# arianna011/Audio-ResiDual

Hardware: NVIDIA B200
Metric: htsat_residual_clips_per_sec (higher is better)
Workload: dtype bf16

## Files before the change

### audio_residual_b200/csrc/ard_common.cuh

```cuda
#pragma once
#include <cuda_runtime.h>
#include <cuda_bf16.h>
#include <cuda_fp16.h>
#include <cuda.h>
#include <stdint.h>

#define ARD_DEVINL __device__ __forceinline__

namespace ard {

ARD_DEVINL uint32_t smem_u32(const void* p) { return static_cast<uint32_t>(__cvta_generic_to_shared(p)); }

ARD_DEVINL uint32_t elect_one_sync() {
    uint32_t pred = 0;
    asm volatile(
        "{\n\t.reg .pred P1;\n\t.reg .b32 R1;\n\t"
        "elect.sync R1|P1, 0xffffffff;\n\t"
        "selp.u32 %0, 1, 0, P1;\n\t}\n"
        : "=r"(pred));
    return pred;
}

ARD_DEVINL uint32_t pack_bf16x2(float lo, float hi) {
    uint32_t r;
// ... 145 lines not shown
}

constexpr uint32_t PAIR_LEADER_MASK = 0xFEFFFFFFu;
ARD_DEVINL uint32_t cluster_ctarank() {
    uint32_t r;
    asm volatile("mov.u32 %0, %%cluster_ctarank;" : "=r"(r));
    return r;
}
ARD_DEVINL void cluster_sync_all() {
    asm volatile("barrier.cluster.arrive.release.aligned;\n\tbarrier.cluster.wait.acquire.aligned;" ::: "memory");
}
ARD_DEVINL void tma_load_2d_pair(void* smem_dst, const CUtensorMap* m, uint64_t* bar, int c0, int c1) {
    asm volatile(
        "cp.async.bulk.tensor.2d.cta_group::2.shared::cluster.global.mbarrier::complete_tx::bytes [%0], [%1, {%3, %4}], [%2];"
        ::"r"(smem_u32(smem_dst)), "l"(reinterpret_cast<uint64_t>(m)), "r"(smem_u32(bar) & PAIR_LEADER_MASK), "r"(c0), "r"(c1)
        : "memory");
}
ARD_DEVINL void tmem_alloc_pair(uint32_t* smem_dst, uint32_t ncols) {
    asm volatile("tcgen05.alloc.cta_group::2.sync.aligned.shared::cta.b32 [%0], %1;" ::"r"(smem_u32(smem_dst)), "r"(ncols)
                 : "memory");
}
ARD_DEVINL void tmem_relinquish_pair() { asm volatile("tcgen05.relinquish_alloc_permit.cta_group::2.sync.aligned;" ::: "memory"); }
ARD_DEVINL void tmem_dealloc_pair(uint32_t taddr, uint32_t ncols) {
    asm volatile("tcgen05.dealloc.cta_group::2.sync.aligned.b32 %0, %1;" ::"r"(taddr), "r"(ncols) : "memory");
}
ARD_DEVINL void umma_bf16_ss_pair(uint32_t tmem_d, uint64_t desc_a, uint64_t desc_b, uint32_t idesc, uint32_t accumulate) {
    asm volatile(
        "{\n\t.reg .pred p;\n\t"
        "setp.ne.b32 p, %4, 0;\n\t"
        "tcgen05.mma.cta_group::2.kind::f16 [%0], %1, %2, %3, p;\n\t}\n"
        ::"r"(tmem_d), "l"(desc_a), "l"(desc_b), "r"(idesc), "r"(accumulate)
        : "memory");
}
ARD_DEVINL void umma_commit_pair(uint64_t* bar) {
    asm volatile("tcgen05.commit.cta_group::2.mbarrier::arrive::one.shared::cluster.multicast::cluster.b64 [%0], %1;"
                 ::"r"(smem_u32(bar)), "h"((uint16_t)3)
                 : "memory");
}
ARD_DEVINL void mbar_arrive_leader(uint64_t* bar) {
    asm volatile("mbarrier.arrive.release.cluster.shared::cluster.b64 _, [%0];" ::"r"(smem_u32(bar) & PAIR_LEADER_MASK) : "memory");
}
ARD_DEVINL void mbar_wait_cluster(uint64_t* bar, uint32_t parity) {
    uint32_t ok = 0;
    while (!ok) {
        asm volatile(
            "{\n\t.reg .pred p;\n\t"
            "mbarrier.try_wait.parity.acquire.cluster.shared::cta.b64 p, [%1], %2;\n\t"
            "selp.u32 %0, 1, 0, p;\n\t}\n"
            : "=r"(ok)
            : "r"(smem_u32(bar)), "r"(parity)
            : "memory");
    }
}

ARD_DEVINL void tmem_ld_32x32b_x32(uint32_t taddr, uint32_t (&v)[32]) {
    asm volatile(
        "tcgen05.ld.sync.aligned.32x32b.x32.b32 "
        "{%0, %1, %2, %3, %4, %5, %6, %7, %8, %9, %10, %11, %12, %13, %14, %15, "
        "%16, %17, %18, %19, %20, %21, %22, %23, %24, %25, %26, %27, %28, %29, %30, %31}, [%32];"
        : "=r"(v[0]), "=r"(v[1]), "=r"(v[2]), "=r"(v[3]), "=r"(v[4]), "=r"(v[5]), "=r"(v[6]), "=r"(v[7]), "=r"(v[8]),
          "=r"(v[9]), "=r"(v[10]), "=r"(v[11]), "=r"(v[12]), "=r"(v[13]), "=r"(v[14]), "=r"(v[15]), "=r"(v[16]),
          "=r"(v[17]), "=r"(v[18]), "=r"(v[19]), "=r"(v[20]), "=r"(v[21]), "=r"(v[22]), "=r"(v[23]), "=r"(v[24]),
          "=r"(v[25]), "=r"(v[26]), "=r"(v[27]), "=r"(v[28]), "=r"(v[29]), "=r"(v[30]), "=r"(v[31])
        : "r"(taddr)
        : "memory");
}
ARD_DEVINL void tmem_ld_32x32b_x16(uint32_t taddr, uint32_t (&v)[16]) {
    asm volatile(
        "tcgen05.ld.sync.aligned.32x32b.x16.b32 "
        "{%0, %1, %2, %3, %4, %5, %6, %7, %8, %9, %10, %11, %12, %13, %14, %15}, [%16];"
        : "=r"(v[0]), "=r"(v[1]), "=r"(v[2]), "=r"(v[3]), "=r"(v[4]), "=r"(v[5]), "=r"(v[6]), "=r"(v[7]), "=r"(v[8]),
          "=r"(v[9]), "=r"(v[10]), "=r"(v[11]), "=r"(v[12]), "=r"(v[13]), "=r"(v[14]), "=r"(v[15])
        : "r"(taddr)
        : "memory");
}
ARD_DEVINL void tmem_ld_32x32b_x8(uint32_t taddr, uint32_t (&v)[8]) {
    asm volatile("tcgen05.ld.sync.aligned.32x32b.x8.b32 {%0, %1, %2, %3, %4, %5, %6, %7}, [%8];"
                 : "=r"(v[0]), "=r"(v[1]), "=r"(v[2]), "=r"(v[3]), "=r"(v[4]), "=r"(v[5]), "=r"(v[6]), "=r"(v[7])
                 : "r"(taddr)
                 : "memory");
}
ARD_DEVINL void tmem_ld_wait() { asm volatile("tcgen05.wait::ld.sync.aligned;" ::: "memory"); }

ARD_DEVINL uint64_t umma_desc_sw128(uint32_t smem_addr) {
    uint64_t d = 0;
    d |= (uint64_t)((smem_addr & 0x3FFFF) >> 4);
    d |= (uint64_t)1 << 16;
    d |= (uint64_t)(1024 >> 4) << 32;
    d |= (uint64_t)1 << 46;
    d |= (uint64_t)2 << 61;
    return d;
}
ARD_DEVINL uint64_t umma_desc_sw64(uint32_t smem_addr) {
    uint64_t d = 0;
    d |= (uint64_t)((smem_addr & 0x3FFFF) >> 4);
    d |= (uint64_t)1 << 16;
    d |= (uint64_t)(512 >> 4) << 32;
    d |= (uint64_t)1 << 46;
    d |= (uint64_t)4 << 61;
    return d;
}
__host__ __device__ constexpr uint32_t umma_idesc_bf16(int M, int N) {
    return (1u << 4) | (1u << 7) | (1u << 10) | ((uint32_t)(N >> 3) << 17) | ((uint32_t)(M >> 4) << 24);
}
__host__ __device__ constexpr uint32_t umma_idesc_f16(int M, int N) {
    return (1u << 4) | ((uint32_t)(N >> 3) << 17) | ((uint32_t)(M >> 4) << 24);
// ... 48 lines not shown
```

### audio_residual_b200/csrc/ffn_wide.cu

```cuda
#include "ard_common.cuh"
#include "ard_internal.h"

namespace ard {

#ifdef ARD_FFN_TRACE
__device__ long long g_ffw_trace[8][64][8];
#define FW_TRACE(role, idx, field) do { if (blockIdx.x == 0 && (idx) < 64) g_ffw_trace[role][idx][field] = clock64(); } while (0)
#else
#define FW_TRACE(role, idx, field) do { } while (0)
#endif

constexpr int FW_BM = 128;
constexpr int FW_EPI_WARPS = 8;
constexpr int FW_GELU_WARPS = 16;
constexpr int FW_W_MMA = FW_EPI_WARPS, FW_W_TMA = FW_W_MMA + 1, FW_W_GELU = FW_W_TMA + 1, FW_W_MMA2 = FW_W_GELU + FW_GELU_WARPS;
constexpr int FW_THREADS = (FW_W_MMA2 + 1) * 32;
constexpr int FW_TM_H = 384;

template <int C>
struct FwCfg {
    static_assert(C == 128 || C == 192 || C == 256 || C == 384, "ffn_wide: C = 128, 192, 256 or 384");
    static constexpr int HD = 4 * C;
    static constexpr int NCH = HD / 64;
    static constexpr int YW = (C % 192 == 0) ? 192 : C;
    static constexpr int KBS = YW / 64;
    static constexpr int SLOT = YW * 128;
    static constexpr int NS = C / YW;
    static constexpr int KB1 = C / 64;
    static constexpr int NYB = 1;
    static constexpr bool A2T = C <= 256;
    static constexpr int TM_A2 = C;
    static constexpr int NA1 = 1;
    static constexpr int NSLOT = C == 128 ? 8 : C == 192 ? 5 : 3;
    static constexpr int A1_KB = FW_BM * 128;
    static constexpr int A1_OFF = 0;
    static constexpr int A1_BYTES = KB1 * A1_KB;
    static constexpr int A2_OFF = A1_OFF + NA1 * A1_BYTES;
    static constexpr int A2_BYTES = FW_BM * 128;
    static constexpr int RING_OFF = A2_OFF + 2 * A2_BYTES;
    static constexpr int CST_OFF = RING_OFF + NSLOT * SLOT;
    static constexpr int VEC_OFF = CST_OFF + FW_EPI_WARPS * 2048;
    static constexpr int BAR_OFF = VEC_OFF + 3 * C * 4;
    static constexpr int SMEM_BYTES = BAR_OFF + 384 + 1024;
    static_assert(SMEM_BYTES <= 227 * 1024, "ffn_wide: shared memory budget");
    static constexpr int LN_CH = C / 16;
    static constexpr int LN_V4 = LN_CH / 4;
    static constexpr int LN_STEPS = LN_CH <= 12 ? 4 : 2;
};

struct FwParams {
    const float* x;
    const float* resid2;
    const float* gamma;
    const float* beta;
    const float* b1h;
    const float* b2;
    int M;
};

template <int C>
__global__ void __launch_bounds__(FW_THREADS, 1)
ffn_wide_kernel(const __grid_constant__ CUtensorMap tmW1, const __grid_constant__ CUtensorMap tmW2,
                const __grid_constant__ CUtensorMap tmOut, const __grid_constant__ CUtensorMap tmX,
                const __grid_constant__ CUtensorMap tmR2, const FwParams p) {
    using Cfg = FwCfg<C>;
    constexpr int NCH = Cfg::NCH, NS = Cfg::NS, NSLOT = Cfg::NSLOT, NYB = Cfg::NYB, NA1 = Cfg::NA1;
    extern __shared__ uint8_t smem_raw[];
    uint8_t* smem = smem_raw + ((1024u - (smem_u32(smem_raw) & 1023u)) & 1023u);
    float* b2s = reinterpret_cast<float*>(smem + Cfg::VEC_OFF);
    float* gs = b2s + C;
    float* bs = gs + C;
    uint64_t* bars = reinterpret_cast<uint64_t*>(smem + Cfg::BAR_OFF);
    uint64_t* ring_full = bars + 0;
    uint64_t* ring_empty = bars + 8;
    uint64_t* a1_full = bars + 16;
    uint64_t* a1_free = bars + 18;
    uint64_t* h_full = bars + 20;
    uint64_t* h_free = bars + 22;
    uint64_t* a2_full = bars + 24;
    uint64_t* a2_free = bars + 26;
    uint64_t* y_full = bars + 28;
    uint64_t* y_free = bars + 30;
    uint32_t* tmem_ptr_smem = reinterpret_cast<uint32_t*>(bars + 32);
    uint64_t* rbar = bars + 34;

    pdl_launch_dependents();
    const int warp = threadIdx.x >> 5, lane = threadIdx.x & 31;
    const int num_tiles = (p.M + FW_BM - 1) / FW_BM;
    const int my_tiles = (num_tiles - (int)blockIdx.x + (int)gridDim.x - 1) / (int)gridDim.x;

    for (int i = threadIdx.x; i < C; i += FW_THREADS) {
        b2s[i] = p.b2[i];
        gs[i] = p.gamma[i];
        bs[i] = p.beta[i];
    }
    if (warp == FW_W_MMA && lane == 0) {
        tma_prefetch_desc(&tmW1);
        tma_prefetch_desc(&tmW2);
        tma_prefetch_desc(&tmOut);
        for (int i = 0; i < NSLOT; ++i) {
            mbar_init(&ring_full[i], 1);
            mbar_init(&ring_empty[i], 1);
        }
        for (int i = 0; i < 2; ++i) {
            mbar_init(&a1_full[i], FW_GELU_WARPS);
            mbar_init(&a1_free[i], 1);
            mbar_init(&h_full[i], 1);
            mbar_init(&h_free[i], FW_GELU_WARPS / 2);
            mbar_init(&a2_full[i], FW_GELU_WARPS / 2);
            mbar_init(&a2_free[i], 1);
            mbar_init(&y_full[i], 1);
            mbar_init(&y_free[i], FW_EPI_WARPS);
        }
        for (int i = 0; i < FW_EPI_WARPS; ++i) mbar_init(&rbar[i], 1);
        fence_barrier_init();
    }
    if (warp == FW_W_MMA) {
        tmem_alloc(tmem_ptr_smem, 512);
        tmem_relinquish();
    }
    tc_fence_before();
    __syncthreads();
    tc_fence_after();
    const uint32_t tmem_base = *tmem_ptr_smem;
    pdl_wait();

    if (warp < FW_EPI_WARPS) {
        constexpr int NCC = C / 32;
        const int quad = warp & 3, c_begin = (warp >> 2) * NCC;
        uint8_t* sbuf = smem + Cfg::CST_OFF + warp * 2048;
        const bool has_r2 = p.resid2 != nullptr;
        if constexpr (Cfg::A2T) {
            uint8_t* rb1 = smem + Cfg::A2_OFF + warp * 4096;
            uint8_t* rb2 = rb1 + 2048;
            auto fetch_resid = [&](int tile, int c) {
                mbar_expect_tx(&rbar[warp], has_r2 ? 4096 : 2048);
                tma_load_2d(rb1, &tmX, &rbar[warp], c * 16, tile * FW_BM + quad * 32);
                if (has_r2) tma_load_2d(rb2, &tmR2, &rbar[warp], c * 16, tile * FW_BM + quad * 32);
            };
            if (lane == 0) fetch_resid(blockIdx.x, c_begin);
            int it = 0;
            for (int tile = blockIdx.x; tile < num_tiles; tile += gridDim.x, ++it) {
                if (warp == 0 && lane == 0) FW_TRACE(0, it, 0);
                mbar_wait_parked(&y_full[0], (uint32_t)(it & 1));
                if (warp == 0 && lane == 0) FW_TRACE(0, it, 1);
                tc_fence_after();
#pragma unroll 1
                for (int cc = 0; cc < NCC; ++cc) {
                    const int c = c_begin + cc;
                    uint32_t v[16];
                    tmem_ld_32x32b_x16(tmem_base + c * 16 + ((uint32_t)(quad * 32) << 16), v);
                    mbar_wait(&rbar[warp], (uint32_t)((it * NCC + cc) & 1));
                    const int sw = (lane >> 1) & 3;
                    float4 r1[4], r2[4];
#pragma unroll
                    for (int j = 0; j < 4; ++j) {
                        r1[j] = *reinterpret_cast<const float4*>(rb1 + lane * 64 + ((j ^ sw) << 4));
                        r2[j] = has_r2 ? *reinterpret_cast<const float4*>(rb2 + lane * 64 + ((j ^ sw) << 4)) : make_float4(0.f, 0.f, 0.f, 0.f);
                    }
                    fence_proxy_async_smem();
                    __syncwarp();
                    if (lane == 0) {
                        if (cc + 1 < NCC) fetch_resid(tile, c + 1);
                        else if (tile + (int)gridDim.x < num_tiles) fetch_resid(tile + gridDim.x, c_begin);
                    }
                    tmem_ld_wait();
                    if (cc == NCC - 1) {
                        tc_fence_before();
                        __syncwarp();
                        if (lane == 0) mbar_arrive(&y_free[0]);
                    }
                    float4 o[4];
#pragma unroll
                    for (int j = 0; j < 4; ++j) {
                        const float4 b4 = *reinterpret_cast<const float4*>(b2s + c * 16 + j * 4);
                        o[j].x = __uint_as_float(v[j * 4 + 0]) + b4.x + r1[j].x + r2[j].x;
                        o[j].y = __uint_as_float(v[j * 4 + 1]) + b4.y + r1[j].y + r2[j].y;
                        o[j].z = __uint_as_float(v[j * 4 + 2]) + b4.z + r1[j].z + r2[j].z;
                        o[j].w = __uint_as_float(v[j * 4 + 3]) + b4.w + r1[j].w + r2[j].w;
                    }
                    if (lane == 0) tma_store_wait_read<0>();
                    __syncwarp();
                    uint8_t* rowp = sbuf + lane * 64;
#pragma unroll
                    for (int j = 0; j < 4; ++j) *reinterpret_cast<float4*>(rowp + ((j ^ sw) << 4)) = o[j];
                    fence_proxy_async_smem();
                    __syncwarp();
                    if (lane == 0) {
                        tma_store_2d(&tmOut, sbuf, c * 16, tile * FW_BM + quad * 32);
                        tma_store_commit();
                    }
                }
                if (warp == 0 && lane == 0) FW_TRACE(0, it, 2);
            }
        } else {
        int it = 0;
        for (int tile = blockIdx.x; tile < num_tiles; tile += gridDim.x, ++it) {
            const int yb = it % NYB;
            const uint32_t ypar = (it / NYB) & 1;
            const long long row = (long long)tile * FW_BM + quad * 32 + lane;
            const bool row_ok = row < p.M;
            float4 r1[4], r2[4];
            auto load_resid = [&](int c) {
#pragma unroll
                for (int j = 0; j < 4; ++j) { r1[j] = make_float4(0.f, 0.f, 0.f, 0.f); r2[j] = r1[j]; }
                if (row_ok) {
                    const float4* rp = reinterpret_cast<const float4*>(p.x + row * C + c * 16);
#pragma unroll
                    for (int j = 0; j < 4; ++j) r1[j] = rp[j];
                    if (has_r2) {
                        const float4* rq = reinterpret_cast<const float4*>(p.resid2 + row * C + c * 16);
#pragma unroll
                        for (int j = 0; j < 4; ++j) r2[j] = rq[j];
                    }
                }
            };
            load_resid(c_begin);
            if (warp == 0 && lane == 0) FW_TRACE(0, it, 0);
            mbar_wait_parked(&y_full[yb], ypar);
            if (warp == 0 && lane == 0) FW_TRACE(0, it, 1);
            tc_fence_after();
#pragma unroll 1
            for (int cc = 0; cc < NCC; ++cc) {
                const int c = c_begin + cc;
                uint32_t v[16];
                tmem_ld_32x32b_x16(tmem_base + yb * 192 + c * 16 + ((uint32_t)(quad * 32) << 16), v);
                tmem_ld_wait();
                if (cc == NCC - 1) {
                    tc_fence_before();
                    __syncwarp();
                    if (lane == 0) mbar_arrive(&y_free[yb]);
                }
                float4 o[4];
#pragma unroll
                for (int j = 0; j < 4; ++j) {
                    const float4 b4 = *reinterpret_cast<const float4*>(b2s + c * 16 + j * 4);
                    o[j].x = __uint_as_float(v[j * 4 + 0]) + b4.x + r1[j].x + r2[j].x;
                    o[j].y = __uint_as_float(v[j * 4 + 1]) + b4.y + r1[j].y + r2[j].y;
                    o[j].z = __uint_as_float(v[j * 4 + 2]) + b4.z + r1[j].z + r2[j].z;
                    o[j].w = __uint_as_float(v[j * 4 + 3]) + b4.w + r1[j].w + r2[j].w;
                }
                if (cc + 1 < NCC) load_resid(c + 1);
                if (lane == 0) tma_store_wait_read<0>();
                __syncwarp();
                uint8_t* rowp = sbuf + lane * 64;
                const int sw = (lane >> 1) & 3;
#pragma unroll
                for (int j = 0; j < 4; ++j) *reinterpret_cast<float4*>(rowp + ((j ^ sw) << 4)) = o[j];
                fence_proxy_async_smem();
                __syncwarp();
                if (lane == 0) {
                    tma_store_2d(&tmOut, sbuf, c * 16, tile * FW_BM + quad * 32);
                    tma_store_commit();
                }
            }
            if (warp == 0 && lane == 0) FW_TRACE(0, it, 2);
        }
        }
        if (lane == 0) tma_store_wait_all<0>();
    } else if (warp == FW_W_TMA) {
        long long n = 0;
        for (int t = 0; t < my_tiles; ++t) {
#pragma unroll 1
            for (int e = 0; e < 2 * NCH; ++e) {
                const bool is_w2 = e >= 2 && (e == 2 * NCH - 1 || (e & 1) == 0);
                const int j = e < 2 ? e : (e == 2 * NCH - 1 ? NCH - 1 : (is_w2 ? (e - 2) >> 1 : (e + 1) >> 1));
#pragma unroll 1
                for (int s = 0; s < NS; ++s, ++n) {
                    const int slot = (int)(n % NSLOT);
                    const uint32_t par = (uint32_t)((n / NSLOT) & 1);
                    if (lane == 0) FW_TRACE(6, (int)n, 0);
                    mbar_wait_parked(&ring_empty[slot], par ^ 1);
                    if (lane == 0) FW_TRACE(6, (int)n, 1);
                    if (elect_one_sync()) {
                        uint8_t* dst = smem + Cfg::RING_OFF + slot * Cfg::SLOT;
                        mbar_expect_tx(&ring_full[slot], Cfg::SLOT);
                        if (is_w2) {
                            tma_load_2d(dst, &tmW2, &ring_full[slot], j * 64, s * Cfg::YW);
                        } else {
#pragma unroll
                            for (int kb = 0; kb < Cfg::KBS; ++kb)
                                tma_load_2d(dst + kb * 8192, &tmW1, &ring_full[slot], s * Cfg::YW + kb * 64, j * 64);
                        }
                    }
                    __syncwarp();
                }
            }
        }
    } else if (warp == FW_W_MMA) {
        constexpr uint32_t idesc1 = umma_idesc_bf16(FW_BM, 64);
        const uint64_t dA1 = umma_desc_sw128(smem_u32(smem + Cfg::A1_OFF));
        const uint32_t ring_u32 = smem_u32(smem + Cfg::RING_OFF);
        long long g = 0;
        for (int t = 0; t < my_tiles; ++t) {
            const int ab = t % NA1;
            mbar_wait_parked(&a1_full[ab], (uint32_t)((t / NA1) & 1));
#pragma unroll 1
            for (int j = 0; j < NCH; ++j, ++g) {
                const int hb = j & 1;
                if (lane == 0) FW_TRACE(1, (int)g, 0);
                mbar_wait_parked(&h_free[hb], (uint32_t)(((g >> 1) & 1) ^ 1));
                if (lane == 0) FW_TRACE(1, (int)g, 1);
                tc_fence_after();
                const int e = j < 2 ? j : 2 * j - 1;
                const long long n0 = ((long long)t * 2 * NCH + e) * NS;
#pragma unroll 1
                for (int s = 0; s < NS; ++s) {
                    const long long n = n0 + s;
                    const int slot = (int)(n % NSLOT);
                    mbar_wait_parked(&ring_full[slot], (uint32_t)((n / NSLOT) & 1));
                    tc_fence_after();
                    if (elect_one_sync()) {
                        const uint32_t d = tmem_base + FW_TM_H + hb * 64;
                        const uint64_t db = umma_desc_sw128(ring_u32 + slot * Cfg::SLOT);
#pragma unroll
                        for (int kb = 0; kb < Cfg::KBS; ++kb)
                            umma_f16_ss_run<4>(d, dA1 + (uint64_t)((ab * Cfg::KB1 + s * Cfg::KBS + kb) * (Cfg::A1_KB >> 4)), db + (uint64_t)(kb * (8192 >> 4)), idesc1,
                                               (s | kb) != 0);
                        umma_commit(&ring_empty[slot]);
                        if (s == NS - 1) {
                            umma_commit(&h_full[hb]);
                            if (j == NCH - 1) umma_commit(&a1_free[ab]);
                        }
                    }
                    __syncwarp();
                    if (lane == 0) FW_TRACE(1, (int)g, 2 + s);
                }
            }
        }
    } else if (warp == FW_W_MMA2) {
        constexpr uint32_t idesc2 = umma_idesc_f16(FW_BM, Cfg::YW);
        const uint64_t dA2 = umma_desc_sw128(smem_u32(smem + Cfg::A2_OFF));
        const uint32_t ring_u32 = smem_u32(smem + Cfg::RING_OFF);
        long long g = 0;
        for (int t = 0; t < my_tiles; ++t) {
            const int yb = t % NYB;
#pragma unroll 1
            for (int j = 0; j < NCH; ++j, ++g) {
                const int b = j & 1;
                if (lane == 0) FW_TRACE(2, (int)g, 0);
                mbar_wait_parked(&a2_full[b], (uint32_t)((g >> 1) & 1));
                if (lane == 0) FW_TRACE(2, (int)g, 1);
                if (j == 0) mbar_wait_parked(&y_free[yb], (uint32_t)(((t / NYB) & 1) ^ 1));
                if (lane == 0) FW_TRACE(2, (int)g, 2);
                tc_fence_after();
                const int e = j < NCH - 1 ? 2 * j + 2 : 2 * NCH - 1;
                const long long n0 = ((long long)t * 2 * NCH + e) * NS;
#pragma unroll 1
                for (int s = 0; s < NS; ++s) {
                    const long long n = n0 + s;
                    const int slot = (int)(n % NSLOT);
                    mbar_wait_parked(&ring_full[slot], (uint32_t)((n / NSLOT) & 1));
                    tc_fence_after();
                    if (elect_one_sync()) {
                        if constexpr (Cfg::A2T)
                            umma_f16_ts_run4(tmem_base + yb * 192 + s * Cfg::YW, tmem_base + Cfg::TM_A2 + b * 32,
                                             umma_desc_sw128(ring_u32 + slot * Cfg::SLOT), idesc2, j != 0);
                        else
                            umma_f16_ss_run<4>(tmem_base + yb * 192 + s * Cfg::YW, dA2 + (uint64_t)(b * (Cfg::A2_BYTES >> 4)),
                                               umma_desc_sw128(ring_u32 + slot * Cfg::SLOT), idesc2, j != 0);
                        umma_commit(&ring_empty[slot]);
                        if (s == NS - 1) {
                            umma_commit(&a2_free[b]);
                            if (j == NCH - 1) umma_commit(&y_full[yb]);
                        }
                    }
                    __syncwarp();
                    if (lane == 0) FW_TRACE(2, (int)g, 3 + s);
                }
            }
        }
    } else {
        const int ew = warp - FW_W_GELU;
        const int quad = warp & 3;
        const int grp = ew >> 3;
        const int half = (ew >> 2) & 1;
        const int row = quad * 32 + lane;
        const int l16 = lane & 15, rsub = lane >> 4;
        uint8_t* a1 = smem + Cfg::A1_OFF;
        auto prefetch_tile = [&](int tile) {
            if (tile >= num_tiles) return;
            const long long r0 = (long long)tile * FW_BM + ew * 8;
            for (int ofs = lane * 128; ofs < 8 * C * 4; ofs += 32 * 128) {
                if ((r0 * C) * 4 + ofs + 128 > (long long)p.M * C * 4) break;
                asm volatile("prefetch.global.L2 [%0];" ::"l"(reinterpret_cast<const char*>(p.x + r0 * C) + ofs));
                if (p.resid2 != nullptr)
                    asm volatile("prefetch.global.L2 [%0];" ::"l"(reinterpret_cast<const char*>(p.resid2 + r0 * C) + ofs));
            }
        };
        auto layernorm_tile = [&](int tile, int lt) {
            prefetch_tile(tile + gridDim.x);
            constexpr int V4 = Cfg::LN_V4, STEPS = Cfg::LN_STEPS;
            bool waited = false;
#pragma unroll 1
            for (int sp = 0; sp < 4 / STEPS; ++sp) {
                float4 v[STEPS][V4];
#pragma unroll
                for (int st = 0; st < STEPS; ++st) {
                    const long long r = (long long)tile * FW_BM + ew * 8 + (sp * STEPS + st) * 2 + rsub;
                    if (r < p.M) {
                        const float4* xr = reinterpret_cast<const float4*>(p.x + r * C + l16 * Cfg::LN_CH);
#pragma unroll
                        for (int q = 0; q < V4; ++q) v[st][q] = __ldg(xr + q);
                    } else {
#pragma unroll
                        for (int q = 0; q < V4; ++q) v[st][q] = make_float4(0.f, 0.f, 0.f, 0.f);
                    }
                }
                if (!waited) {
                    if (ew == 0 && lane == 0) FW_TRACE(3, lt, 0);
                    mbar_wait_parked(&a1_free[lt % NA1], (uint32_t)(((lt / NA1) & 1) ^ 1));
                    if (ew == 0 && lane == 0) FW_TRACE(3, lt, 1);
                    waited = true;
                }
                float sm[STEPS], qv[STEPS];
#pragma unroll
                for (int st = 0; st < STEPS; ++st) {
                    sm[st] = 0.f;
#pragma unroll
                    for (int q = 0; q < V4; ++q) sm[st] += (v[st][q].x + v[st][q].y) + (v[st][q].z + v[st][q].w);
                }
#pragma unroll
                for (int sh = 8; sh > 0; sh >>= 1)
#pragma unroll
                    for (int st = 0; st < STEPS; ++st) sm[st] += __shfl_xor_sync(0xffffffffu, sm[st], sh);
#pragma unroll
                for (int st = 0; st < STEPS; ++st) {
                    const float mean = sm[st] * (1.0f / C);
                    qv[st] = 0.f;
#pragma unroll
                    for (int q = 0; q < V4; ++q) {
                        v[st][q].x -= mean; v[st][q].y -= mean; v[st][q].z -= mean; v[st][q].w -= mean;
                        qv[st] += (v[st][q].x * v[st][q].x + v[st][q].y * v[st][q].y) + (v[st][q].z * v[st][q].z + v[st][q].w * v[st][q].w);
                    }
                }
#pragma unroll
                for (int sh = 8; sh > 0; sh >>= 1)
#pragma unroll
                    for (int st = 0; st < STEPS; ++st) qv[st] += __shfl_xor_sync(0xffffffffu, qv[st], sh);
#pragma unroll
                for (int st = 0; st < STEPS; ++st) {
                    const float rstd = rsqrtf(qv[st] * (1.0f / C) + 1e-5f);
                    const int rr = ew * 8 + (sp * STEPS + st) * 2 + rsub;
#pragma unroll
                    for (int q = 0; q < V4; ++q) {
                        const int c0 = l16 * Cfg::LN_CH + q * 4;
                        const float4 gm = *reinterpret_cast<const float4*>(gs + c0);
                        const float4 bt = *reinterpret_cast<const float4*>(bs + c0);
                        uint2 pk;
                        pk.x = pack_bf16x2(fmaf(v[st][q].x * rstd, gm.x, bt.x), fmaf(v[st][q].y * rstd, gm.y, bt.y));
                        pk.y = pack_bf16x2(fmaf(v[st][q].z * rstd, gm.z, bt.z), fmaf(v[st][q].w * rstd, gm.w, bt.w));
                        const int kb = c0 >> 6, cc = c0 & 63;
                        *reinterpret_cast<uint2*>(a1 + ((lt % NA1) * Cfg::KB1 + kb) * Cfg::A1_KB + rr * 128 + (((cc >> 3) ^ (rr & 7)) << 4) + (cc & 7) * 2) = pk;
                    }
                }
            }
            fence_proxy_async_smem();
            __syncwarp();
            if (lane == 0) mbar_arrive(&a1_full[lt % NA1]);
            if (ew == 0 && lane == 0) FW_TRACE(3, lt, 2);
        };

        prefetch_tile(blockIdx.x);
        if (my_tiles > 0) layernorm_tile(blockIdx.x, 0);
        int it = 0;
        for (int tile = blockIdx.x; tile < num_tiles; tile += gridDim.x, ++it) {
#pragma unroll 1
            for (int jj = 0; jj < NCH / 2; ++jj) {
                const int j = 2 * jj + grp;
                const long long g = (long long)it * NCH + j;
                if ((ew & 7) == 0 && lane == 0) FW_TRACE(4 + grp, (int)g, 0);
                mbar_wait_parked(&h_full[grp], (uint32_t)((g >> 1) & 1));
                if ((ew & 7) == 0 && lane == 0) FW_TRACE(4 + grp, (int)g, 1);
                tc_fence_after();
                uint32_t pk[16];
#pragma unroll
                for (int s = 0; s < 2; ++s) {
                    uint32_t v[16];
                    tmem_ld_32x32b_x16(tmem_base + FW_TM_H + grp * 64 + half * 32 + s * 16 + ((uint32_t)(quad * 32) << 16), v);
                    const float* bb = p.b1h + j * 64 + half * 32 + s * 16;
                    float4 b4[4];
#pragma unroll
                    for (int i = 0; i < 4; ++i) b4[i] = __ldg(reinterpret_cast<const float4*>(bb) + i);
                    tmem_ld_wait();
                    if (s == 1) {
                        tc_fence_before();
                        __syncwarp();
                        if (lane == 0) mbar_arrive(&h_free[grp]);
                    }
#pragma unroll
                    for (int i = 0; i < 16; i += 4) {
                        const float4 hb4 = b4[i >> 2];
                        pk[s * 8 + i / 2] = gelu_erf_f16x2_halved(fmaf(__uint_as_float(v[i]), 0.5f, hb4.x), fmaf(__uint_as_float(v[i + 1]), 0.5f, hb4.y));
                        pk[s * 8 + i / 2 + 1] = gelu_erf_f16x2_halved(fmaf(__uint_as_float(v[i + 2]), 0.5f, hb4.z), fmaf(__uint_as_float(v[i + 3]), 0.5f, hb4.w));
                    }
                }
                if ((ew & 7) == 0 && lane == 0) FW_TRACE(4 + grp, (int)g, 2);
                mbar_wait_parked(&a2_free[grp], (uint32_t)(((g >> 1) & 1) ^ 1));
                tc_fence_after();
                if ((ew & 7) == 0 && lane == 0) FW_TRACE(4 + grp, (int)g, 3);
                if constexpr (Cfg::A2T) {
                    tmem_st_32x32b_x16(tmem_base + Cfg::TM_A2 + grp * 32 + half * 16 + ((uint32_t)(quad * 32) << 16), pk);
                    tmem_st_wait();
                    tc_fence_before();
                } else {
                    uint8_t* rowp = smem + Cfg::A2_OFF + grp * Cfg::A2_BYTES + row * 128;
                    const int sw = row & 7;
#pragma unroll
                    for (int q = 0; q < 4; ++q)
                        *reinterpret_cast<uint4*>(rowp + (((half * 4 + q) ^ sw) << 4)) = make_uint4(pk[q * 4], pk[q * 4 + 1], pk[q * 4 + 2], pk[q * 4 + 3]);
                    fence_proxy_async_smem();
                }
                __syncwarp();
                if (lane == 0) mbar_arrive(&a2_full[grp]);
                if ((ew & 7) == 0 && lane == 0) FW_TRACE(4 + grp, (int)g, 4);
                if (NA1 == 2 && jj == grp && tile + (int)gridDim.x < num_tiles) layernorm_tile(tile + gridDim.x, it + 1);
            }
            if (NA1 == 1 && tile + (int)gridDim.x < num_tiles) layernorm_tile(tile + gridDim.x, it + 1);
        }
    }

    tc_fence_before();
    __syncthreads();
    if (warp == FW_W_MMA) {
        tc_fence_after();
        tmem_dealloc(tmem_base, 512);
    }
}

template <int C>
static int launch_ffn_wide(const float* x, const float* resid2, float* out, long long M, const float* gamma, const float* beta,
                           const __nv_bfloat16* w1, const float* b1_half, const __half* w2_f16, const float* b2, int num_sms, cudaStream_t stream) {
    using Cfg = FwCfg<C>;
    CUtensorMap t1, t2, to;
    ARD_TRY(make_tmap_2d(&t1, w1, 2, C, Cfg::HD, (uint64_t)C * 2, 64, 64, 128));
    ARD_TRY(make_tmap_2d(&t2, w2_f16, 2, Cfg::HD, C, (uint64_t)Cfg::HD * 2, 64, Cfg::YW, 128));
    ARD_TRY(make_tmap_2d(&to, out, 4, C, (uint64_t)M, (uint64_t)C * 4, 16, 32, 64));
    CUtensorMap tx, tr;
    ARD_TRY(make_tmap_2d(&tx, x, 4, C, (uint64_t)M, (uint64_t)C * 4, 16, 32, 64));
    ARD_TRY(make_tmap_2d(&tr, resid2 ? resid2 : x, 4, C, (uint64_t)M, (uint64_t)C * 4, 16, 32, 64));
    static bool attr_set = false;
    if (!attr_set) {
        ARD_CUDA(cudaFuncSetAttribute(ffn_wide_kernel<C>, cudaFuncAttributeMaxDynamicSharedMemorySize, Cfg::SMEM_BYTES));
        attr_set = true;
    }
    FwParams p;
    p.x = x; p.resid2 = resid2; p.gamma = gamma; p.beta = beta; p.b1h = b1_half; p.b2 = b2; p.M = (int)M;
    const int tiles = (int)((M + FW_BM - 1) / FW_BM);
    const int grid = tiles < num_sms ? tiles : num_sms;
    const double MC = (double)M * C;
    ProfScope ps(PROF_FFN, stream, 2.0 * M * C * Cfg::HD * 2.0, MC * 4.0 * (2.0 + (resid2 ? 1.0 : 0.0)) + 2.0 * 2.0 * C * Cfg::HD);
    ARD_CUDA(enqueue_pdl(ffn_wide_kernel<C>, dim3(grid), dim3(FW_THREADS), Cfg::SMEM_BYTES, stream, t1, t2, to, tx, tr, p));
    return check_cuda(cudaGetLastError(), "ffn_wide launch");
}

int ffn_fused_wide(const float* x, const float* resid2, float* out, long long M, int C, const float* gamma, const float* beta,
                   const __nv_bfloat16* w1, const float* b1_half, const __half* w2_f16, const float* b2, int num_sms, cudaStream_t stream) {
    if (M <= 0) return 0;
    if (M > 0x7fffffffLL) return set_error(ARD_ERR_SHAPE, "ffn_wide: too many rows");
    if (C == 128) return launch_ffn_wide<128>(x, resid2, out, M, gamma, beta, w1, b1_half, w2_f16, b2, num_sms, stream);
    if (C == 192) return launch_ffn_wide<192>(x, resid2, out, M, gamma, beta, w1, b1_half, w2_f16, b2, num_sms, stream);
    if (C == 256) return launch_ffn_wide<256>(x, resid2, out, M, gamma, beta, w1, b1_half, w2_f16, b2, num_sms, stream);
    if (C == 384) return launch_ffn_wide<384>(x, resid2, out, M, gamma, beta, w1, b1_half, w2_f16, b2, num_sms, stream);
    return set_error(ARD_ERR_SHAPE, "ffn_wide: C = %d not supported (128, 192, 256, 384)", C);
}

}

#ifdef ARD_FFN_TRACE
extern "C" int ard_debug_ffw_trace(long long* host_out) {
    return (int)cudaMemcpyFromSymbol(host_out, ard::g_ffw_trace, sizeof(long long) * 8 * 64 * 8);
}
#endif
```

Before: 25270.

## Run C=384 fused FFN on 2-CTA clusters with paired UMMA and TMA residuals

The C=384 fused FFN now runs on CTA pairs. Each pair processes a 256-row tile with cta_group::2 UMMA, multicast-style paired TMA weight loads that split each ring slot across the two CTAs, cluster-scoped barriers and paired TMEM allocation. Only the leader CTA issues MMAs. This is meant to halve the per-CTA weight traffic and shared-memory footprint for the widest stage. The register-based residual epilogue used for C=384 is also replaced with TMA-prefetched residual tiles in extra shared memory. The cost is cross-CTA synchronization and half as many independent schedulers.

```diff
diff --git a/audio_residual_b200/csrc/ard_common.cuh b/audio_residual_b200/csrc/ard_common.cuh
--- a/audio_residual_b200/csrc/ard_common.cuh
+++ b/audio_residual_b200/csrc/ard_common.cuh
@@ -221,6 +221,18 @@
             : "memory");
     }
 }
+ARD_DEVINL void mbar_wait_cluster_parked(uint64_t* bar, uint32_t parity) {
+    uint32_t ok = 0;
+    while (!ok) {
+        asm volatile(
+            "{\n\t.reg .pred p;\n\t"
+            "mbarrier.try_wait.parity.acquire.cluster.shared::cta.b64 p, [%1], %2, %3;\n\t"
+            "selp.u32 %0, 1, 0, p;\n\t}\n"
+            : "=r"(ok)
+            : "r"(smem_u32(bar)), "r"(parity), "r"(0x989680u)
+            : "memory");
+    }
+}
 
 ARD_DEVINL void tmem_ld_32x32b_x32(uint32_t taddr, uint32_t (&v)[32]) {
     asm volatile(
diff --git a/audio_residual_b200/csrc/ffn_wide.cu b/audio_residual_b200/csrc/ffn_wide.cu
--- a/audio_residual_b200/csrc/ffn_wide.cu
+++ b/audio_residual_b200/csrc/ffn_wide.cu
@@ -17,18 +17,23 @@
 constexpr int FW_THREADS = (FW_W_MMA2 + 1) * 32;
 constexpr int FW_TM_H = 384;
 
-template <int C>
+template <int C, bool PAIR>
 struct FwCfg {
     static_assert(C == 128 || C == 192 || C == 256 || C == 384, "ffn_wide: C = 128, 192, 256 or 384");
+    static_assert(PAIR == (C == 384), "ffn_wide: C = 384 runs on CTA pairs, the other widths on single CTAs");
+    static constexpr int TILE_M = PAIR ? 2 * FW_BM : FW_BM;
     static constexpr int HD = 4 * C;
     static constexpr int NCH = HD / 64;
     static constexpr int YW = (C % 192 == 0) ? 192 : C;
     static constexpr int KBS = YW / 64;
-    static constexpr int SLOT = YW * 128;
+    static constexpr int W1KB = (PAIR ? 32 : 64) * 128;
+    static constexpr int SLOT = (PAIR ? YW / 2 : YW) * 128;
     static constexpr int NS = C / YW;
+    static_assert(KBS * W1KB == SLOT, "ffn_wide: ring slot layout");
     static constexpr int KB1 = C / 64;
     static constexpr int NYB = 1;
     static constexpr bool A2T = C <= 256;
+    static constexpr bool TMA_RESID = A2T || PAIR;
     static constexpr int TM_A2 = C;
     static constexpr int NA1 = 1;
     static constexpr int NSLOT = C == 128 ? 8 : C == 192 ? 5 : 3;
@@ -39,7 +44,8 @@
     static constexpr int A2_BYTES = FW_BM * 128;
     static constexpr int RING_OFF = A2_OFF + 2 * A2_BYTES;
     static constexpr int CST_OFF = RING_OFF + NSLOT * SLOT;
-    static constexpr int VEC_OFF = CST_OFF + FW_EPI_WARPS * 2048;
+    static constexpr int RB_OFF = A2T ? A2_OFF : CST_OFF + FW_EPI_WARPS * 2048;
+    static constexpr int VEC_OFF = CST_OFF + FW_EPI_WARPS * 2048 + (A2T ? 0 : FW_EPI_WARPS * 4096);
     static constexpr int BAR_OFF = VEC_OFF + 3 * C * 4;
     static constexpr int SMEM_BYTES = BAR_OFF + 384 + 1024;
     static_assert(SMEM_BYTES <= 227 * 1024, "ffn_wide: shared memory budget");
@@ -58,13 +64,13 @@
     int M;
 };
 
-template <int C>
+template <int C, bool PAIR>
 __global__ void __launch_bounds__(FW_THREADS, 1)
 ffn_wide_kernel(const __grid_constant__ CUtensorMap tmW1, const __grid_constant__ CUtensorMap tmW2,
                 const __grid_constant__ CUtensorMap tmOut, const __grid_constant__ CUtensorMap tmX,
                 const __grid_constant__ CUtensorMap tmR2, const FwParams p) {
-    using Cfg = FwCfg<C>;
-    constexpr int NCH = Cfg::NCH, NS = Cfg::NS, NSLOT = Cfg::NSLOT, NYB = Cfg::NYB, NA1 = Cfg::NA1;
+    using Cfg = FwCfg<C, PAIR>;
+    constexpr int NCH = Cfg::NCH, NS = Cfg::NS, NSLOT = Cfg::NSLOT, NYB = Cfg::NYB, NA1 = Cfg::NA1, TILE_M = Cfg::TILE_M;
     extern __shared__ uint8_t smem_raw[];
     uint8_t* smem = smem_raw + ((1024u - (smem_u32(smem_raw) & 1023u)) & 1023u);
     float* b2s = reinterpret_cast<float*>(smem + Cfg::VEC_OFF);
@@ -86,8 +92,24 @@
 
     pdl_launch_dependents();
     const int warp = threadIdx.x >> 5, lane = threadIdx.x & 31;
-    const int num_tiles = (p.M + FW_BM - 1) / FW_BM;
-    const int my_tiles = (num_tiles - (int)blockIdx.x + (int)gridDim.x - 1) / (int)gridDim.x;
+    const uint32_t rank = PAIR ? (blockIdx.x & 1u) : 0u;
+    const int sched_id = PAIR ? (int)(blockIdx.x >> 1) : (int)blockIdx.x;
+    const int sched_n = PAIR ? (int)(gridDim.x >> 1) : (int)gridDim.x;
+    const int num_tiles = (p.M + TILE_M - 1) / TILE_M;
+    const int my_tiles = (num_tiles - sched_id + sched_n - 1) / sched_n;
+    auto row_base = [&](int tile) { return (long long)tile * TILE_M + (int)rank * FW_BM; };
+    auto arrive_issuer = [&](uint64_t* b) {
+        if constexpr (PAIR) mbar_arrive_leader(b);
+        else mbar_arrive(b);
+    };
+    auto wait_both = [&](uint64_t* b, uint32_t parity) {
+        if constexpr (PAIR) mbar_wait_cluster_parked(b, parity);
+        else mbar_wait_parked(b, parity);
+    };
+    auto commit = [&](uint64_t* b) {
+        if constexpr (PAIR) umma_commit_pair(b);
+        else umma_commit(b);
+    };
 
     for (int i = threadIdx.x; i < C; i += FW_THREADS) {
         b2s[i] = p.b2[i];
@@ -102,25 +124,32 @@
             mbar_init(&ring_full[i], 1);
             mbar_init(&ring_empty[i], 1);
         }
+        constexpr uint32_t NCTA = PAIR ? 2 : 1;
         for (int i = 0; i < 2; ++i) {
-            mbar_init(&a1_full[i], FW_GELU_WARPS);
+            mbar_init(&a1_full[i], NCTA * FW_GELU_WARPS);
             mbar_init(&a1_free[i], 1);
             mbar_init(&h_full[i], 1);
-            mbar_init(&h_free[i], FW_GELU_WARPS / 2);
-            mbar_init(&a2_full[i], FW_GELU_WARPS / 2);
+            mbar_init(&h_free[i], NCTA * FW_GELU_WARPS / 2);
+            mbar_init(&a2_full[i], NCTA * FW_GELU_WARPS / 2);
             mbar_init(&a2_free[i], 1);
             mbar_init(&y_full[i], 1);
-            mbar_init(&y_free[i], FW_EPI_WARPS);
+            mbar_init(&y_free[i], NCTA * FW_EPI_WARPS);
         }
         for (int i = 0; i < FW_EPI_WARPS; ++i) mbar_init(&rbar[i], 1);
         fence_barrier_init();
     }
     if (warp == FW_W_MMA) {
-        tmem_alloc(tmem_ptr_smem, 512);
-        tmem_relinquish();
+        if constexpr (PAIR) {
+            tmem_alloc_pair(tmem_ptr_smem, 512);
+            tmem_relinquish_pair();
+        } else {
+            tmem_alloc(tmem_ptr_smem, 512);
+            tmem_relinquish();
+        }
     }
     tc_fence_before();
-    __syncthreads();
+    if constexpr (PAIR) cluster_sync_all();
+    else __syncthreads();
     tc_fence_after();
     const uint32_t tmem_base = *tmem_ptr_smem;
     pdl_wait();
@@ -130,17 +159,20 @@
         const int quad = warp & 3, c_begin = (warp >> 2) * NCC;
         uint8_t* sbuf = smem + Cfg::CST_OFF + warp * 2048;
         const bool has_r2 = p.resid2 != nullptr;
-        if constexpr (Cfg::A2T) {
-            uint8_t* rb1 = smem + Cfg::A2_OFF + warp * 4096;
+        static_assert(Cfg::TMA_RESID, "ffn_wide: every width prefetches its residual tiles by TMA");
+        {
+            uint8_t* rb1 = smem + Cfg::RB_OFF + warp * 4096;
             uint8_t* rb2 = rb1 + 2048;
             auto fetch_resid = [&](int tile, int c) {
                 mbar_expect_tx(&rbar[warp], has_r2 ? 4096 : 2048);
-                tma_load_2d(rb1, &tmX, &rbar[warp], c * 16, tile * FW_BM + quad * 32);
-                if (has_r2) tma_load_2d(rb2, &tmR2, &rbar[warp], c * 16, tile * FW_BM + quad * 32);
+                const int r0 = tile * TILE_M + (int)rank * FW_BM + quad * 32;
+                tma_load_2d(rb1, &tmX, &rbar[warp], c * 16, r0);
+                if (has_r2) tma_load_2d(rb2, &tmR2, &rbar[warp], c * 16, r0);
             };
-            if (lane == 0) fetch_resid(blockIdx.x, c_begin);
+            if (lane == 0) fetch_resid(sched_id, c_begin);
             int it = 0;
-            for (int tile = blockIdx.x; tile < num_tiles; tile += gridDim.x, ++it) {
+            for (int tile = sched_id; tile < num_tiles; tile += sched_n, ++it) {
+                const int row0 = tile * TILE_M + (int)rank * FW_BM + quad * 32;
                 if (warp == 0 && lane == 0) FW_TRACE(0, it, 0);
                 mbar_wait_parked(&y_full[0], (uint32_t)(it & 1));
                 if (warp == 0 && lane == 0) FW_TRACE(0, it, 1);
@@ -162,13 +194,13 @@
                     __syncwarp();
                     if (lane == 0) {
                         if (cc + 1 < NCC) fetch_resid(tile, c + 1);
-                        else if (tile + (int)gridDim.x < num_tiles) fetch_resid(tile + gridDim.x, c_begin);
+                        else if (tile + sched_n < num_tiles) fetch_resid(tile + sched_n, c_begin);
                     }
                     tmem_ld_wait();
                     if (cc == NCC - 1) {
                         tc_fence_before();
                         __syncwarp();
-                        if (lane == 0) mbar_arrive(&y_free[0]);
+                        if (lane == 0) arrive_issuer(&y_free[0]);
                     }
                     float4 o[4];
 #pragma unroll
@@ -186,76 +218,13 @@
                     for (int j = 0; j < 4; ++j) *reinterpret_cast<float4*>(rowp + ((j ^ sw) << 4)) = o[j];
                     fence_proxy_async_smem();
                     __syncwarp();
-                    if (lane == 0) {
-                        tma_store_2d(&tmOut, sbuf, c * 16, tile * FW_BM + quad * 32);
+                    if (lane == 0 && (!PAIR || row0 < p.M)) {
+                        tma_store_2d(&tmOut, sbuf, c * 16, row0);
                         tma_store_commit();
                     }
                 }
                 if (warp == 0 && lane == 0) FW_TRACE(0, it, 2);
             }
-        } else {
-        int it = 0;
-        for (int tile = blockIdx.x; tile < num_tiles; tile += gridDim.x, ++it) {
-            const int yb = it % NYB;
-            const uint32_t ypar = (it / NYB) & 1;
-            const long long row = (long long)tile * FW_BM + quad * 32 + lane;
-            const bool row_ok = row < p.M;
-            float4 r1[4], r2[4];
-            auto load_resid = [&](int c) {
-#pragma unroll
-                for (int j = 0; j < 4; ++j) { r1[j] = make_float4(0.f, 0.f, 0.f, 0.f); r2[j] = r1[j]; }
-                if (row_ok) {
-                    const float4* rp = reinterpret_cast<const float4*>(p.x + row * C + c * 16);
-#pragma unroll
-                    for (int j = 0; j < 4; ++j) r1[j] = rp[j];
-                    if (has_r2) {
-                        const float4* rq = reinterpret_cast<const float4*>(p.resid2 + row * C + c * 16);
-#pragma unroll
-                        for (int j = 0; j < 4; ++j) r2[j] = rq[j];
-                    }
-                }
-            };
-            load_resid(c_begin);
-            if (warp == 0 && lane == 0) FW_TRACE(0, it, 0);
-            mbar_wait_parked(&y_full[yb], ypar);
-            if (warp == 0 && lane == 0) FW_TRACE(0, it, 1);
-            tc_fence_after();
-#pragma unroll 1
-            for (int cc = 0; cc < NCC; ++cc) {
-                const int c = c_begin + cc;
-                uint32_t v[16];
-                tmem_ld_32x32b_x16(tmem_base + yb * 192 + c * 16 + ((uint32_t)(quad * 32) << 16), v);
-                tmem_ld_wait();
-                if (cc == NCC - 1) {
-                    tc_fence_before();
-                    __syncwarp();
-                    if (lane == 0) mbar_arrive(&y_free[yb]);
-                }
-                float4 o[4];
-#pragma unroll
-                for (int j = 0; j < 4; ++j) {
-                    const float4 b4 = *reinterpret_cast<const float4*>(b2s + c * 16 + j * 4);
-                    o[j].x = __uint_as_float(v[j * 4 + 0]) + b4.x + r1[j].x + r2[j].x;
-                    o[j].y = __uint_as_float(v[j * 4 + 1]) + b4.y + r1[j].y + r2[j].y;
-                    o[j].z = __uint_as_float(v[j * 4 + 2]) + b4.z + r1[j].z + r2[j].z;
-                    o[j].w = __uint_as_float(v[j * 4 + 3]) + b4.w + r1[j].w + r2[j].w;
-                }
-                if (cc + 1 < NCC) load_resid(c + 1);
-                if (lane == 0) tma_store_wait_read<0>();
-                __syncwarp();
-                uint8_t* rowp = sbuf + lane * 64;
-                const int sw = (lane >> 1) & 3;
-#pragma unroll
-                for (int j = 0; j < 4; ++j) *reinterpret_cast<float4*>(rowp + ((j ^ sw) << 4)) = o[j];
-                fence_proxy_async_smem();
-                __syncwarp();
-                if (lane == 0) {
-                    tma_store_2d(&tmOut, sbuf, c * 16, tile * FW_BM + quad * 32);
-                    tma_store_commit();
-                }
-            }
-            if (warp == 0 && lane == 0) FW_TRACE(0, it, 2);
-        }
         }
         if (lane == 0) tma_store_wait_all<0>();
     } else if (warp == FW_W_TMA) {
@@ -274,32 +243,43 @@
                     if (lane == 0) FW_TRACE(6, (int)n, 1);
                     if (elect_one_sync()) {
                         uint8_t* dst = smem + Cfg::RING_OFF + slot * Cfg::SLOT;
-                        mbar_expect_tx(&ring_full[slot], Cfg::SLOT);
-                        if (is_w2) {
-                            tma_load_2d(dst, &tmW2, &ring_full[slot], j * 64, s * Cfg::YW);
+                        if constexpr (PAIR) {
+                            if (rank == 0) mbar_expect_tx(&ring_full[slot], 2 * Cfg::SLOT);
+                            if (is_w2) {
+                                tma_load_2d_pair(dst, &tmW2, &ring_full[slot], j * 64, s * Cfg::YW + (int)rank * (Cfg::YW / 2));
+                            } else {
+#pragma unroll
+                                for (int kb = 0; kb < Cfg::KBS; ++kb)
+                                    tma_load_2d_pair(dst + kb * Cfg::W1KB, &tmW1, &ring_full[slot], s * Cfg::YW + kb * 64, j * 64 + (int)rank * 32);
+                            }
                         } else {
-#pragma unroll
-                            for (int kb = 0; kb < Cfg::KBS; ++kb)
-                                tma_load_2d(dst + kb * 8192, &tmW1, &ring_full[slot], s * Cfg::YW + kb * 64, j * 64);
+                            mbar_expect_tx(&ring_full[slot], Cfg::SLOT);
+                            if (is_w2) {
+                                tma_load_2d(dst, &tmW2, &ring_full[slot], j * 64, s * Cfg::YW);
+                            } else {
+#pragma unroll
+                                for (int kb = 0; kb < Cfg::KBS; ++kb)
+                                    tma_load_2d(dst + kb * Cfg::W1KB, &tmW1, &ring_full[slot], s * Cfg::YW + kb * 64, j * 64);
+                            }
                         }
                     }
                     __syncwarp();
                 }
             }
         }
-    } else if (warp == FW_W_MMA) {
-        constexpr uint32_t idesc1 = umma_idesc_bf16(FW_BM, 64);
+    } else if (warp == FW_W_MMA && rank == 0) {
+        constexpr uint32_t idesc1 = umma_idesc_bf16(TILE_M, 64);
         const uint64_t dA1 = umma_desc_sw128(smem_u32(smem + Cfg::A1_OFF));
         const uint32_t ring_u32 = smem_u32(smem + Cfg::RING_OFF);
         long long g = 0;
         for (int t = 0; t < my_tiles; ++t) {
             const int ab = t % NA1;
-            mbar_wait_parked(&a1_full[ab], (uint32_t)((t / NA1) & 1));
+            wait_both(&a1_full[ab], (uint32_t)((t / NA1) & 1));
 #pragma unroll 1
             for (int j = 0; j < NCH; ++j, ++g) {
                 const int hb = j & 1;
                 if (lane == 0) FW_TRACE(1, (int)g, 0);
-                mbar_wait_parked(&h_free[hb], (uint32_t)(((g >> 1) & 1) ^ 1));
+                wait_both(&h_free[hb], (uint32_t)(((g >> 1) & 1) ^ 1));
                 if (lane == 0) FW_TRACE(1, (int)g, 1);
                 tc_fence_after();
                 const int e = j < 2 ? j : 2 * j - 1;
@@ -315,12 +295,12 @@
                         const uint64_t db = umma_desc_sw128(ring_u32 + slot * Cfg::SLOT);
 #pragma unroll
                         for (int kb = 0; kb < Cfg::KBS; ++kb)
-                            umma_f16_ss_run<4>(d, dA1 + (uint64_t)((ab * Cfg::KB1 + s * Cfg::KBS + kb) * (Cfg::A1_KB >> 4)), db + (uint64_t)(kb * (8192 >> 4)), idesc1,
-                                               (s | kb) != 0);
-                        umma_commit(&ring_empty[slot]);
+                            umma_f16_ss_run<4, PAIR>(d, dA1 + (uint64_t)((ab * Cfg::KB1 + s * Cfg::KBS + kb) * (Cfg::A1_KB >> 4)),
+                                                     db + (uint64_t)(kb * (Cfg::W1KB >> 4)), idesc1, (s | kb) != 0);
+                        commit(&ring_empty[slot]);
                         if (s == NS - 1) {
-                            umma_commit(&h_full[hb]);
-                            if (j == NCH - 1) umma_commit(&a1_free[ab]);
+                            commit(&h_full[hb]);
+                            if (j == NCH - 1) commit(&a1_free[ab]);
                         }
                     }
                     __syncwarp();
@@ -328,8 +308,8 @@
                 }
             }
         }
-    } else if (warp == FW_W_MMA2) {
-        constexpr uint32_t idesc2 = umma_idesc_f16(FW_BM, Cfg::YW);
+    } else if (warp == FW_W_MMA2 && rank == 0) {
+        constexpr uint32_t idesc2 = umma_idesc_f16(TILE_M, Cfg::YW);
         const uint64_t dA2 = umma_desc_sw128(smem_u32(smem + Cfg::A2_OFF));
         const uint32_t ring_u32 = smem_u32(smem + Cfg::RING_OFF);
         long long g = 0;
@@ -339,9 +319,9 @@
             for (int j = 0; j < NCH; ++j, ++g) {
                 const int b = j & 1;
                 if (lane == 0) FW_TRACE(2, (int)g, 0);
-                mbar_wait_parked(&a2_full[b], (uint32_t)((g >> 1) & 1));
+                wait_both(&a2_full[b], (uint32_t)((g >> 1) & 1));
                 if (lane == 0) FW_TRACE(2, (int)g, 1);
-                if (j == 0) mbar_wait_parked(&y_free[yb], (uint32_t)(((t / NYB) & 1) ^ 1));
+                if (j == 0) wait_both(&y_free[yb], (uint32_t)(((t / NYB) & 1) ^ 1));
                 if (lane == 0) FW_TRACE(2, (int)g, 2);
                 tc_fence_after();
                 const int e = j < NCH - 1 ? 2 * j + 2 : 2 * NCH - 1;
@@ -357,12 +337,12 @@
                             umma_f16_ts_run4(tmem_base + yb * 192 + s * Cfg::YW, tmem_base + Cfg::TM_A2 + b * 32,
                                              umma_desc_sw128(ring_u32 + slot * Cfg::SLOT), idesc2, j != 0);
                         else
-                            umma_f16_ss_run<4>(tmem_base + yb * 192 + s * Cfg::YW, dA2 + (uint64_t)(b * (Cfg::A2_BYTES >> 4)),
-                                               umma_desc_sw128(ring_u32 + slot * Cfg::SLOT), idesc2, j != 0);
-                        umma_commit(&ring_empty[slot]);
+                            umma_f16_ss_run<4, PAIR>(tmem_base + yb * 192 + s * Cfg::YW, dA2 + (uint64_t)(b * (Cfg::A2_BYTES >> 4)),
+                                                     umma_desc_sw128(ring_u32 + slot * Cfg::SLOT), idesc2, j != 0);
+                        commit(&ring_empty[slot]);
                         if (s == NS - 1) {
-                            umma_commit(&a2_free[b]);
-                            if (j == NCH - 1) umma_commit(&y_full[yb]);
+                            commit(&a2_free[b]);
+                            if (j == NCH - 1) commit(&y_full[yb]);
                         }
                     }
                     __syncwarp();
@@ -370,6 +350,7 @@
                 }
             }
         }
+    } else if (warp == FW_W_MMA || warp == FW_W_MMA2) {
     } else {
         const int ew = warp - FW_W_GELU;
         const int quad = warp & 3;
@@ -380,7 +361,7 @@
         uint8_t* a1 = smem + Cfg::A1_OFF;
         auto prefetch_tile = [&](int tile) {
             if (tile >= num_tiles) return;
-            const long long r0 = (long long)tile * FW_BM + ew * 8;
+            const long long r0 = row_base(tile) + ew * 8;
             for (int ofs = lane * 128; ofs < 8 * C * 4; ofs += 32 * 128) {
                 if ((r0 * C) * 4 + ofs + 128 > (long long)p.M * C * 4) break;
                 asm volatile("prefetch.global.L2 [%0];" ::"l"(reinterpret_cast<const char*>(p.x + r0 * C) + ofs));
@@ -389,7 +370,7 @@
             }
         };
         auto layernorm_tile = [&](int tile, int lt) {
-            prefetch_tile(tile + gridDim.x);
+            prefetch_tile(tile + sched_n);
             constexpr int V4 = Cfg::LN_V4, STEPS = Cfg::LN_STEPS;
             bool waited = false;
 #pragma unroll 1
@@ -397,7 +378,7 @@
                 float4 v[STEPS][V4];
 #pragma unroll
                 for (int st = 0; st < STEPS; ++st) {
-                    const long long r = (long long)tile * FW_BM + ew * 8 + (sp * STEPS + st) * 2 + rsub;
+                    const long long r = row_base(tile) + ew * 8 + (sp * STEPS + st) * 2 + rsub;
                     if (r < p.M) {
                         const float4* xr = reinterpret_cast<const float4*>(p.x + r * C + l16 * Cfg::LN_CH);
 #pragma unroll
@@ -457,14 +438,14 @@
             }
             fence_proxy_async_smem();
             __syncwarp();
-            if (lane == 0) mbar_arrive(&a1_full[lt % NA1]);
+            if (lane == 0) arrive_issuer(&a1_full[lt % NA1]);
             if (ew == 0 && lane == 0) FW_TRACE(3, lt, 2);
         };
 
-        prefetch_tile(blockIdx.x);
-        if (my_tiles > 0) layernorm_tile(blockIdx.x, 0);
+        prefetch_tile(sched_id);
+        if (my_tiles > 0) layernorm_tile(sched_id, 0);
         int it = 0;
-        for (int tile = blockIdx.x; tile < num_tiles; tile += gridDim.x, ++it) {
+        for (int tile = sched_id; tile < num_tiles; tile += sched_n, ++it) {
 #pragma unroll 1
             for (int jj = 0; jj < NCH / 2; ++jj) {
                 const int j = 2 * jj + grp;
@@ -486,7 +467,7 @@
                     if (s == 1) {
                         tc_fence_before();
                         __syncwarp();
-                        if (lane == 0) mbar_arrive(&h_free[grp]);
+                        if (lane == 0) arrive_issuer(&h_free[grp]);
                     }
 #pragma unroll
                     for (int i = 0; i < 16; i += 4) {
@@ -512,56 +493,77 @@
                     fence_proxy_async_smem();
                 }
                 __syncwarp();
-                if (lane == 0) mbar_arrive(&a2_full[grp]);
+                if (lane == 0) arrive_issuer(&a2_full[grp]);
                 if ((ew & 7) == 0 && lane == 0) FW_TRACE(4 + grp, (int)g, 4);
-                if (NA1 == 2 && jj == grp && tile + (int)gridDim.x < num_tiles) layernorm_tile(tile + gridDim.x, it + 1);
-            }
-            if (NA1 == 1 && tile + (int)gridDim.x < num_tiles) layernorm_tile(tile + gridDim.x, it + 1);
+                if (NA1 == 2 && jj == grp && tile + sched_n < num_tiles) layernorm_tile(tile + sched_n, it + 1);
+            }
+            if (NA1 == 1 && tile + sched_n < num_tiles) layernorm_tile(tile + sched_n, it + 1);
         }
     }
 
     tc_fence_before();
-    __syncthreads();
+    if constexpr (PAIR) cluster_sync_all();
+    else __syncthreads();
     if (warp == FW_W_MMA) {
         tc_fence_after();
-        tmem_dealloc(tmem_base, 512);
+        if constexpr (PAIR) tmem_dealloc_pair(tmem_base, 512);
+        else tmem_dealloc(tmem_base, 512);
     }
 }
 
-template <int C>
+template <int C, bool PAIR>
 static int launch_ffn_wide(const float* x, const float* resid2, float* out, long long M, const float* gamma, const float* beta,
                            const __nv_bfloat16* w1, const float* b1_half, const __half* w2_f16, const float* b2, int num_sms, cudaStream_t stream) {
-    using Cfg = FwCfg<C>;
+    using Cfg = FwCfg<C, PAIR>;
     CUtensorMap t1, t2, to;
-    ARD_TRY(make_tmap_2d(&t1, w1, 2, C, Cfg::HD, (uint64_t)C * 2, 64, 64, 128));
-    ARD_TRY(make_tmap_2d(&t2, w2_f16, 2, Cfg::HD, C, (uint64_t)Cfg::HD * 2, 64, Cfg::YW, 128));
+    ARD_TRY(make_tmap_2d(&t1, w1, 2, C, Cfg::HD, (uint64_t)C * 2, 64, Cfg::W1KB / 128, 128));
+    ARD_TRY(make_tmap_2d(&t2, w2_f16, 2, Cfg::HD, C, (uint64_t)Cfg::HD * 2, 64, Cfg::SLOT / 128, 128));
     ARD_TRY(make_tmap_2d(&to, out, 4, C, (uint64_t)M, (uint64_t)C * 4, 16, 32, 64));
     CUtensorMap tx, tr;
     ARD_TRY(make_tmap_2d(&tx, x, 4, C, (uint64_t)M, (uint64_t)C * 4, 16, 32, 64));
     ARD_TRY(make_tmap_2d(&tr, resid2 ? resid2 : x, 4, C, (uint64_t)M, (uint64_t)C * 4, 16, 32, 64));
+    auto kern = ffn_wide_kernel<C, PAIR>;
     static bool attr_set = false;
     if (!attr_set) {
-        ARD_CUDA(cudaFuncSetAttribute(ffn_wide_kernel<C>, cudaFuncAttributeMaxDynamicSharedMemorySize, Cfg::SMEM_BYTES));
+        ARD_CUDA(cudaFuncSetAttribute(kern, cudaFuncAttributeMaxDynamicSharedMemorySize, Cfg::SMEM_BYTES));
         attr_set = true;
     }
     FwParams p;
     p.x = x; p.resid2 = resid2; p.gamma = gamma; p.beta = beta; p.b1h = b1_half; p.b2 = b2; p.M = (int)M;
-    const int tiles = (int)((M + FW_BM - 1) / FW_BM);
-    const int grid = tiles < num_sms ? tiles : num_sms;
+    const int tiles = (int)((M + Cfg::TILE_M - 1) / Cfg::TILE_M);
     const double MC = (double)M * C;
     ProfScope ps(PROF_FFN, stream, 2.0 * M * C * Cfg::HD * 2.0, MC * 4.0 * (2.0 + (resid2 ? 1.0 : 0.0)) + 2.0 * 2.0 * C * Cfg::HD);
-    ARD_CUDA(enqueue_pdl(ffn_wide_kernel<C>, dim3(grid), dim3(FW_THREADS), Cfg::SMEM_BYTES, stream, t1, t2, to, tx, tr, p));
-    return check_cuda(cudaGetLastError(), "ffn_wide launch");
+    if constexpr (PAIR) {
+        const int pairs = tiles < num_sms / 2 ? tiles : num_sms / 2;
+        cudaLaunchConfig_t cfg = {};
+        cfg.gridDim = dim3(2 * pairs);
+        cfg.blockDim = dim3(FW_THREADS);
+        cfg.dynamicSmemBytes = Cfg::SMEM_BYTES;
+        cfg.stream = stream;
+        cudaLaunchAttribute at[2];
+        at[0].id = cudaLaunchAttributeClusterDimension;
+        at[0].val.clusterDim.x = 2; at[0].val.clusterDim.y = 1; at[0].val.clusterDim.z = 1;
+        at[1].id = cudaLaunchAttributeProgrammaticStreamSerialization;
+        at[1].val.programmaticStreamSerializationAllowed = 1;
+        cfg.attrs = at;
+        cfg.numAttrs = pdl_enabled() ? 2 : 1;
+        ARD_CUDA(cudaLaunchKernelEx(&cfg, kern, t1, t2, to, tx, tr, p));
+        return check_cuda(cudaGetLastError(), "ffn_wide pair launch");
+    } else {
+        const int grid = tiles < num_sms ? tiles : num_sms;
+        ARD_CUDA(enqueue_pdl(kern, dim3(grid), dim3(FW_THREADS), Cfg::SMEM_BYTES, stream, t1, t2, to, tx, tr, p));
+        return check_cuda(cudaGetLastError(), "ffn_wide launch");
+    }
 }
 
 int ffn_fused_wide(const float* x, const float* resid2, float* out, long long M, int C, const float* gamma, const float* beta,
                    const __nv_bfloat16* w1, const float* b1_half, const __half* w2_f16, const float* b2, int num_sms, cudaStream_t stream) {
     if (M <= 0) return 0;
     if (M > 0x7fffffffLL) return set_error(ARD_ERR_SHAPE, "ffn_wide: too many rows");
-    if (C == 128) return launch_ffn_wide<128>(x, resid2, out, M, gamma, beta, w1, b1_half, w2_f16, b2, num_sms, stream);
-    if (C == 192) return launch_ffn_wide<192>(x, resid2, out, M, gamma, beta, w1, b1_half, w2_f16, b2, num_sms, stream);
-    if (C == 256) return launch_ffn_wide<256>(x, resid2, out, M, gamma, beta, w1, b1_half, w2_f16, b2, num_sms, stream);
-    if (C == 384) return launch_ffn_wide<384>(x, resid2, out, M, gamma, beta, w1, b1_half, w2_f16, b2, num_sms, stream);
+    if (C == 128) return launch_ffn_wide<128, false>(x, resid2, out, M, gamma, beta, w1, b1_half, w2_f16, b2, num_sms, stream);
+    if (C == 192) return launch_ffn_wide<192, false>(x, resid2, out, M, gamma, beta, w1, b1_half, w2_f16, b2, num_sms, stream);
+    if (C == 256) return launch_ffn_wide<256, false>(x, resid2, out, M, gamma, beta, w1, b1_half, w2_f16, b2, num_sms, stream);
+    if (C == 384) return launch_ffn_wide<384, true>(x, resid2, out, M, gamma, beta, w1, b1_half, w2_f16, b2, num_sms, stream);
     return set_error(ARD_ERR_SHAPE, "ffn_wide: C = %d not supported (128, 192, 256, 384)", C);
 }
 
```

After: 25240 (median of 6 runs). No clear change (-0.1%).
